# lalithsuresh/rapid

Hardware: NVIDIA H100
Metric: alert_cells_per_sec_to_converged_cut (higher is better)
Workload: dtype u16

## Files before the change

rapid_b200/csrc/cd_bucketed.cu:

```cuda
#include <cooperative_groups.h>

#include <algorithm>
#include <climits>
#include <cstdlib>

#include "cd_internal.cuh"

namespace cg = cooperative_groups;

namespace rapid {

#ifndef RAPID_UNI_MINBLOCKS
#define RAPID_UNI_MINBLOCKS 5
#endif
#ifndef RAPID_SPLIT_LOOP
#define RAPID_SPLIT_LOOP 0
#endif
#ifndef RAPID_PF
#define RAPID_PF 2
#endif
#ifndef RAPID_INVAL_SPLIT
#define RAPID_INVAL_SPLIT 1
#endif
#ifndef RAPID_PF_L1
// ... 472 lines not shown
                    }
                    s_ne[t] = (uint8_t)ne;
                }
                if (fresh && !edges) {
                    un = (visit_acc<PERM, SEQ>(f, 0u, d, &sw[0], &spw[0], RM, L, H) && block_active) ? 1 : 0;
                    if (PERM) { f.minTH = T32_NONE; f.minTLun = T32_NONE; }
                } else {
                    if (!PERM) sw[t] = a.walk[base + t];
                    if (SEQ) spw[t] = a.pwalk[base + t];
                    if (fresh) s_src[t] = nullptr;
                    if (MEMO && !fresh && !edges && block_active) {
                        const uint32_t sst = rows.get(s_src[t], (int64_t)sample_at);
                        uint32_t at_last = sst;
                        const bool mun = visit_acc<PERM, SEQ>(m, sst & RM, d, &sw[PERM ? 0 : t], &spw[SEQ ? t : 0], RM, L, H, nullptr, 0u, seq_last, &at_last);
                        s_mst[t] = sst;
                        s_mrep[t] = group8_rep<HB>((SEQ ? (at_last | (sst & ~RM)) : sst) | s_nw[t]);
                        s_mun[t] = mun ? 1 : 0;
                        memo = true;
                    }
                }
                if (MEMO) { if (!memo) s_mst[t] = 0xFFFFFFFFu; else s_macc[t] = stage_pack<SEQ>(m); }
                s_unres[t] = (un && a.wl.has_so[d.slot]) ? 1 : 0;
                if (!fresh || edges) s_unres[t] = a.wl.has_so[d.slot] ? 0 : -1;
                heavy = !fresh || edges;
            }
            {
                const unsigned hm = __ballot_sync(0xffffffffu, heavy);
                if (t == 0) s_heavy = __popc(hm);
            }
            const StageAcc fr = stage_reduce<SEQ>(stage_pack<SEQ>(f));
            if (t == 0) chunk_add<SEQ>(s_facc, fr);
// ... 70 lines not shown
                        uint32_t so_st = 0;
                        if (s_erow[i][e]) same = group8_same<HB>(group8_load<HB>(rows, s_erow[i][e], r0), am, &so_st);
                        const int ob = s_eob[i][e], k = s_ek[i][e];
                        const uint32_t bLo = observer_L_batch(so_st & RM, ob >= 0 ? &a.desc[ob] : nullptr, ob >= 0 ? &a.pwalk[ob] : nullptr, L);
                        u[k] = (bLo == T32_NONE || bDown == T32_NONE) ? T32_NONE : max(bLo, bDown);
                        umask |= 1u << k;
                    }
                }
                if (mhit) {
                    hit |= 1u << i;
                    unres = s_mun[i] != 0;
                    group8_merge<HB>(w, s_mrep[i], am);
                } else if (same) {
                    uint32_t at_last = st;
                    unres = visit_acc<PERM, SEQ>(com, st & RM, d, &sw[PERM ? 0 : i], &spw[SEQ ? i : 0], RM, L, H, u, umask, seq_last, &at_last);
                    group8_merge<HB>(w, group8_rep<HB>((SEQ ? (at_last | (st & ~RM)) : st) | s_nw[i]), am);
                } else {
                    if (!had_exc) {
                        had_exc = true;
                        const Acc zero;
#pragma unroll
                        for (int j = 0; j < 8; ++j) part_store<SEQ>(a.part, pbase + j, zero);
                    }
                    const uint32_t nwb = s_nw[i];
#pragma unroll (SEQ ? 1 : 8)
                    for (int j = 0; j < 8; ++j) {
                        if (!((act >> j) & 1u)) continue;
                        const uint32_t sj = group8_word<HB>(w, j);
                        Acc ex;
                        uint32_t at_last = sj;
                        if (SEQ && ne) umask = edge_times(a, d.slot, r0 + j, false, receiver_down_batch(a, ((seen >> j) & 1u) ? RF_SEEN_DOWN : 0u, false), u);
// ... 170 lines not shown
                    if (v.seen_down) fl |= PF_SEEN;
                    if (v.c0 >= L && v.c0 < H) tp++;
                    if (v.crossL) nL++;
                    if (v.crossH) {
                        nH++;
                        if (!haveTH || v.tH < minTH) { minTH = v.tH; haveTH = true; }
                        h1 += d.mix1; h2 += d.mix2;
                    }
                    if (v.c1 >= L && v.c1 < H) {
                        unres = true;
                        if (v.crossL) { nUn++; if (!haveTL || v.tL < minTLun) { minTLun = v.tL; haveTL = true; } }
                        else fl |= PF_NEGINF;
                    }
                    st |= v.have;
                }
                if (a.rows.hb == 4) row_store1_warp<4>(a.rows, s_dst[i], r, st);
                else row_store1_warp<8>(a.rows, s_dst[i], r, st);
            }
            if (__any_sync(0xffffffffu, unres) && (t & 31) == 0 && s_unres[i] == 0) s_unres[i] = 1;
        }
        __syncthreads();
        if (t < n && s_unres[t] > 0) note_unresolved(a, tile, sd[t].slot);
    }
    if (t == 0) {
        if ((blockIdx.x * GEN_THREADS) % TILE_R == 0) a.part.flag[(size_t)chunk * a.part.n_tiles + tile] = 1;
        if (blockIdx.x == 0) a.part.chunk[chunk] = chunk_zero();
    }
    if (r < (int64_t)a.Rpad) {
        const size_t p = (size_t)chunk * a.Rpad + (size_t)r;
        a.part.cnt[p] = make_uint4(nL, nH, tp | (fl << PF_SHIFT), nUn);
        a.part.minTH[p] = minTH;
        a.part.minTLun[p] = minTLun;
        a.part.h1[p] = h1;
        a.part.h2[p] = h2;
    }
}

struct ResolveArgs {
    ApplyArgs ap;
    BatchCounts* bc;
    BatchCounts* snap;
    int n_chunks;
    int uniform;
    int counts_only;
    int seq;
    uint8_t* seq_dev;
    uint8_t* cur_w;
    int32_t* n_pre;
    uint32_t* rflags;
    uint64_t* pend_h1;
    uint64_t* pend_h2;
    int32_t* pend_cnt;
    uint64_t* out_h1;
    uint64_t* out_h2;
// ... 291 lines not shown
    for (int64_t r = (int64_t)blockIdx.x * blockDim.x + threadIdx.x; r < a.ap.R; r += (int64_t)gridDim.x * blockDim.x) {
        const uint32_t fl = a.mx_fl[r];
        if (!((fl & MX_DONE) && (fl & MX_HAS_E))) continue;
        const uint64_t o1 = a.mx_p1[r] + a.mx_e1[r], o2 = a.mx_p2[r] + a.mx_e2[r];
        const int32_t oc = a.mx_pc[r] + a.mx_ec[r];
        a.out_h1[r] = o1; a.out_h2[r] = o2; a.out_len[r] = oc;
        a.pend_h1[r] -= o1; a.pend_h2[r] -= o2; a.pend_cnt[r] -= oc;
        a.mx_e1[r] = 0; a.mx_e2[r] = 0; a.mx_ec[r] = 0;
        a.rflags[r] = (a.rflags[r] | RF_ANNOUNCED | RF_ANN_NOW | RF_MIXED_EMIT) & ~RF_RULE_GE_H;
    }
}

__device__ __noinline__ bool emitted_in_batch(const ResolveArgs& e, int32_t s, int64_t r, uint32_t w_new, uint64_t rs) {
    const ApplyArgs& a = e.ap;
    const uint32_t RM = (1u << a.K) - 1u;
    if (e.touch[s] != e.serial) return __popc(w_new & RM) >= a.H && !(w_new & CD_BIT_CALL);
    const int b = e.batch_index[s];
    const SubjDesc d = a.desc[b];
    const uint32_t old = seq_state(a, d, b, r, (s >= a.bc->S_before ? 0u : a.rows.get(a.rows.alt_lo(s), r)) & RM, true, true);
    if (__popc(old & RM) >= a.H) return true;
    SubjWalk wl;
    if (e.uniform) wl = a.walk[b];
    const IVisit v = interval_visit(a, e.uniform, old & RM, d, &wl, r, rs);
    return v.crossH && v.tH <= e.estar[r];
}

constexpr int INV_STAGE = 128;
struct InvSmem {
    uint8_t* row[INV_STAGE];
    uint64_t mix1[INV_STAGE], mix2[INV_STAGE];
    uint8_t ne[INV_STAGE];
// ... 96 lines not shown
                            miss[j] = (k3[j] && c >= a.L && c < a.H) ? (~w[j] & RM) : 0u;
                            anymiss |= miss[j];
                        }
                        if (!anymiss) continue;
                        uint32_t implicit[4] = {0u, 0u, 0u, 0u};
                        for (int ei = eb; ei < ee; ++ei) {
                            const int k = sm.e_k[ei];
                            if (!((anymiss >> k) & 1u)) continue;
                            const uint2 o2 = ei == eb ? e0v[q] : ei == eb + 1 ? e1v[q] : a.rows.load4(sm.e_row[ei], rb);
                            uint32_t wo[4];
#pragma unroll
                            for (int j = 0; j < 4; ++j) wo[j] = a.rows.word4(o2, j);
#pragma unroll
                            for (int j = 0; j < 4; ++j) {
                                if (!((miss[j] >> k) & 1u)) continue;
                                if ((wo[j] & CD_BIT_EMIT) || __popc(wo[j] & RM) < a.L) continue;
                                if (MX) {
                                    const int64_t r = rb + j;
                                    if (emitted_in_batch(e, sm.e_so[ei], r, wo[j], splitmix64(a.dl.perm_seed + (uint64_t)(a.rbegin + r)))) continue;
                                }
                                implicit[j] |= 1u << k;
                            }
                        }
                        bool any = false;
#pragma unroll
                        for (int j = 0; j < 4; ++j) {
                            if (!implicit[j]) continue;
                            any = true;
                            uint32_t nw = w[j] | implicit[j];
                            const bool raised = __popc(nw & RM) >= a.H;
                            if (raised && mixed) nw |= CD_BIT_CALL;
                            w[j] = nw;
                            if (raised) { ++res[j]; kh1[j] += sm.mix1[i]; kh2[j] += sm.mix2[i]; }
                        }
                        if (any) a.rows.store4(sm.row[i], rb, w);
                    }
                }
            }
        }
#if RAPID_INVAL_SPLIT
        if (P > 1) {
#pragma unroll
            for (int j = 0; j < 4; ++j)
                if (res[j] > 0) { atomicAdd(&e.inv_res[rb + j], res[j]); atomicAdd(&e.inv_h1[rb + j], (unsigned long long)kh1[j]); atomicAdd(&e.inv_h2[rb + j], (unsigned long long)kh2[j]); }
            __threadfence();
            __syncthreads();
            if (t == 0) s_fin = atomicAdd(&e.inv_ticket[tile], 1) == P - 1 ? 1 : 0;
            __syncthreads();
            if (!s_fin) continue;
// ... 31 lines not shown
            if ((flags[j] & RF_MIXED_EMIT) && (flags[j] & RF_ANN_NOW) && !(flags[j] & RF_RULE_GE_H)) ++my_inval;
            ann |= ((flags[j] & RF_ANNOUNCED) ? 1u : 0u) << (8 * j);
        }
        if (touched) {
            *reinterpret_cast<uint4*>(e.rflags + rb) = make_uint4(flags[0], flags[1], flags[2], flags[3]);
            *reinterpret_cast<uint32_t*>(e.out_ann + rb) = ann;
        }
    }
    if (MX) {
        const int32_t b = block_sum_i32(my_inval, s_red);
        if (t == 0 && b) atomicAdd(&e.bc->n_inval, b);
    }
}

__device__ __noinline__ void phase_mixed_mark(const ResolveArgs& e, int32_t S) {
    const ApplyArgs& a = e.ap;
    const int spb = 64;
    const int rblocks = (int)(a.Rpad / GEN_THREADS), sblocks = (S + spb - 1) / spb;
    const int64_t items = (int64_t)rblocks * sblocks;
    for (int64_t wi = blockIdx.x; wi < items; wi += gridDim.x) {
        const int64_t r = (wi % rblocks) * GEN_THREADS + threadIdx.x;
        if (r >= a.R) continue;
        const uint32_t f = e.rflags[r];
        if (!(f & RF_MIXED_EMIT) || !(f & RF_ANN_NOW) || (f & RF_RULE_GE_H)) continue;
        const uint64_t rs = splitmix64(a.dl.perm_seed + (uint64_t)(a.rbegin + r));
        const int32_t s0 = (int32_t)(wi / rblocks) * spb, s1 = min(S, s0 + spb);
        for (int32_t s = s0; s < s1; ++s) {
            uint8_t* row = a.rows.cur_lo(s);
            const uint32_t w = a.rows.get(row, r);
            if (!(w & CD_BIT_EMIT) && emitted_in_batch(e, s, r, w, rs)) a.rows.hi_or(row, r, CD_BIT_EMIT);
        }
    }
}

__device__ void phase_inval_unmark(const ResolveArgs& e) {
    const ApplyArgs& a = e.ap;
    const int n_list = min(*(volatile int32_t*)a.wl.count, a.wl.cap);
    const int64_t items = (int64_t)n_list * a.wl.n_tiles;
    for (int64_t p = blockIdx.x; p < items; p += gridDim.x) {
        const int32_t sl = a.wl.slots[p / a.wl.n_tiles];
        const int tile = (int)(p % a.wl.n_tiles);
        if (!a.wl.in_tile[(size_t)sl * a.wl.n_tiles + tile]) continue;
        uint8_t* row = a.rows.cur_lo(sl);
        for (int q = 0; q < TILE_R / GEN_THREADS; ++q) {
            const int64_t r = (int64_t)tile * TILE_R + q * GEN_THREADS + threadIdx.x;
            if (r >= a.R) continue;
            if (a.rows.get(row, r) & CD_BIT_CALL) a.rows.hi_clear(row, r, CD_BIT_CALL);
        }
    }
}

__device__ void resolve_tail(const ResolveArgs& a, int32_t serial) {
    __shared__ int s_last;
    __syncthreads();
    if (threadIdx.x == 0) {
        __threadfence();
        s_last = atomicAdd(&a.bc->ticket, 1) == (int)gridDim.x - 1;
    }
    __syncthreads();
    if (!s_last || threadIdx.x != 0) return;
    __threadfence();
    volatile BatchCounts* b = a.bc;
    BatchCounts c;
// ... 368 lines not shown
    }
}

int32_t bucketed_apply(CD* cd, int64_t A, const DeliveryDev& dl, bool seq) {
    Bucketed* b = state(cd);
    cudaStream_t s = cd->stream;
    const bool uniform = !(dl.flags & (RAPID_DELIVERY_BITMAP | RAPID_DELIVERY_PERMUTED));
    const bool counts_only = (dl.flags & RAPID_DELIVERY_PERMUTED) && !(dl.flags & RAPID_DELIVERY_BITMAP);
    const bool swar = uniform || counts_only;
    b->n_tiles = (int)(cd->Rpad / TILE_R);

    if (b->slots_uniform == 0) {
        int dev = 0, sms = TARGET_SMS, per_u = 8, per_g = 4, per_r = 2;
        cudaGetDevice(&dev);
        cudaDeviceGetAttribute(&sms, cudaDevAttrMultiProcessorCount, dev);
        cudaOccupancyMaxActiveBlocksPerMultiprocessor(&per_u, k_apply_uniform<false, false, 4>, UNI_THREADS, 0);
        cudaOccupancyMaxActiveBlocksPerMultiprocessor(&per_g, k_apply_generic, GEN_THREADS, 0);
        cudaOccupancyMaxActiveBlocksPerMultiprocessor(&per_r, k_mixed_flip, GEN_THREADS, 0);
        int per_m = 2;
        cudaOccupancyMaxActiveBlocksPerMultiprocessor(&per_m, k_marks, GEN_THREADS, 0);
        per_r = std::min(per_r, per_m);
        b->slots_uniform = sms * std::max(per_u, 1);
        b->slots_generic = sms * std::max(per_g, 1);
        b->resolve_grid = sms * std::max(per_r, 1);
    }
    int Sb = (int)std::max<int64_t>(1, std::min<int64_t>(A, cd->est_A > 0 ? (A * (int64_t)std::max(cd->est_Sb, 1) + cd->est_A - 1) / cd->est_A
                                                                           : (2 * A + cd->K - 1) / cd->K));
    Sb = (int)std::min<int64_t>(Sb, (int64_t)std::max<size_t>(cd->S_cap, 1));
    int n_chunks = 1;
    {
        const int rblocks = swar ? b->n_tiles : (int)(cd->Rpad / GEN_THREADS);
// ... 37 lines not shown
    RAPID_CHECK(b->p_chunk.reserve((size_t)n_chunks));
    Partials part{b->p_cnt.p, b->p_cntp.p, b->p_minTH.p, b->p_minTLun.p, b->p_h1.p, b->p_h2.p, b->p_h1p.p, b->p_h2p.p, b->p_seq.p, b->p_flag.p, b->p_chunk.p, b->n_tiles};

    ApplyArgs ap;
    ap.rows = RowRef{cd->masks.p, cd->cur.p, cd->Rpad, cd->row_stride, cd->nbuf, cd->hb}; ap.Rpad = cd->Rpad;
    ap.K = cd->K; ap.H = cd->H; ap.L = cd->L; ap.R = cd->R; ap.rbegin = cd->rbegin;
    ap.rflags = cd->rflags.p; ap.dl = dl; ap.bc = cd->counts.p;
    ap.desc = b->desc.p; ap.walk = b->walk.p; ap.pwalk = b->pwalk.p; ap.slot_subject = cd->slot_subject.p;
    ap.touch = cd->touch.p; ap.batch_index = b->batch_index.p; ap.serial = cd->batch_serial; ap.seq = seq ? 1 : 0;
    ap.sidx = b->sidx.p; ap.s_ring = b->s_ring.p; ap.s_status = b->s_status.p;
    ap.part = part; ap.n_tiles = b->n_tiles; ap.wl = worklist(b);

    RAPID_CUDA(cudaEventRecord(cd->evk0, s));
    if (swar) {
        dim3 grid((unsigned)b->n_tiles, (unsigned)n_chunks);
        if (cd->hb == 4) launch_uniform<4>(grid, s, ap, counts_only, seq);
        else launch_uniform<8>(grid, s, ap, counts_only, seq);
        cd->last_path = counts_only ? 4 : 2;
    } else {
        dim3 grid((unsigned)(cd->Rpad / GEN_THREADS), (unsigned)n_chunks);
        k_apply_generic<<<grid, GEN_THREADS, 0, s>>>(ap);
        cd->last_path = 3;
    }
    RAPID_KERNEL_CHECK();
    RAPID_CUDA(cudaEventRecord(cd->evk1, s));

    ResolveArgs ra;
    ra.ap = ap; ra.bc = cd->counts.p; ra.snap = cd->counts_snap.p; ra.n_chunks = n_chunks;
    ra.uniform = uniform ? 1 : 0; ra.counts_only = counts_only ? 1 : 0; ra.cur_w = cd->cur.p;
    ra.seq = seq ? 1 : 0; ra.seq_dev = nullptr;
    ra.n_pre = cd->n_pre.p; ra.rflags = cd->rflags.p; ra.pend_h1 = cd->pend_h1.p; ra.pend_h2 = cd->pend_h2.p;
    ra.pend_cnt = cd->pend_cnt.p; ra.out_h1 = cd->out_h1.p; ra.out_h2 = cd->out_h2.p; ra.out_len = cd->out_len.p; ra.out_ann = cd->out_ann.p;
    ra.mx_fl = b->mx_fl.p; ra.mx_a = b->mx_a.p; ra.mx_cand = b->mx_cand.p; ra.mx_emax = b->mx_emax.p;
    ra.mx_p1 = b->mx_p1.p; ra.mx_p2 = b->mx_p2.p; ra.mx_pc = b->mx_pc.p; ra.estar = b->estar.p;
    ra.mx_e1 = b->mx_e1.p; ra.mx_e2 = b->mx_e2.p; ra.mx_ec = b->mx_ec.p; ra.mx_changed = b->mx_changed.p; ra.mx_dev = b->mx_dev.p;
    ra.slot_of = cd->slot_of.p; ra.obs = cd->view->obs.p; ra.touch = cd->touch.p; ra.batch_index = b->batch_index.p;
    ra.serial = cd->batch_serial;
#if RAPID_INVAL_SPLIT
    const int inv_split = b->n_tiles >= 64 ? 1 : std::min(32, (2 * TARGET_SMS + std::max(b->n_tiles, 1) - 1) / std::max(b->n_tiles, 1));
    if (inv_split > 1 && !b->inv_res.p) {
        RAPID_CHECK(b->inv_res.reserve(cd->Rpad)); RAPID_CHECK(b->inv_h1.reserve(cd->Rpad)); RAPID_CHECK(b->inv_h2.reserve(cd->Rpad));
        RAPID_CHECK(b->inv_ticket.reserve((size_t)std::max(b->n_tiles, 1)));
        RAPID_CUDA(cudaMemsetAsync(b->inv_res.p, 0, cd->Rpad * sizeof(int32_t), s));
// ... 35 lines not shown
```

rapid_b200/csrc/cd_core.cu:

```cuda
#include <algorithm>
#include <climits>
#include <cstdio>
#include <cstdlib>

#include "cd_internal.cuh"
#include "radix.cuh"

namespace rapid {

__global__ void k_fill_i32(int32_t* p, int64_t n, int32_t v) {
    const int64_t i = (int64_t)blockIdx.x * blockDim.x + threadIdx.x;
    if (i < n) p[i] = v;
}

struct SweepArgs {
    int K, H, L, raw, do_cells, do_inval;
    int64_t R;
    RowRef rows;
    int32_t S;
    const int32_t* slot_subject;
    const int32_t* slot_of;
    const int32_t* obs;
    int64_t A;
    const int32_t* cell_slot;
// ... 127 lines not shown
    if (w & CD_BIT_CALL) {
        *p = (uint16_t)(w & ~CD_BIT_CALL);
        const int32_t at = atomicAdd(count, 1);
        if (at < cap) out[at] = slot_subject[s];
    }
}
__global__ void k_clear_call(RowRef rows, int32_t S, int64_t R) {
    const int64_t r = (int64_t)blockIdx.x * blockDim.x + threadIdx.x;
    const int32_t s = blockIdx.y;
    if (r >= R || s >= S) return;
    uint16_t* p = rows.row(s) + r;
    const uint32_t w = *p;
    if (w & CD_BIT_CALL) *p = (uint16_t)(w & ~CD_BIT_CALL);
}

__global__ void k_gather_proposal(RowRef rows, int32_t S, int64_t r, int H, uint32_t RM, int rule_ge_h,
                                  const int32_t* __restrict__ slot_subject, const int64_t* __restrict__ key0,
                                  int32_t* __restrict__ out_ids, int64_t* __restrict__ out_keys, int32_t cap,
                                  int32_t* __restrict__ count) {
    const int32_t s = blockIdx.x * blockDim.x + threadIdx.x;
    if (s >= S) return;
    const uint32_t w = rows.get(s, r);
    const bool in = rule_ge_h ? (__popc(w & RM) >= H) : ((w & CD_BIT_EMIT) != 0);
    if (in) {
        const int32_t at = atomicAdd(count, 1);
        if (at < cap) { const int32_t id = slot_subject[s]; out_ids[at] = id; out_keys[at] = key0[id]; }
    }
}

__global__ void k_dump_masks(RowRef rows, int32_t S, int64_t r, uint32_t RM, const int32_t* __restrict__ slot_subject,
                             int32_t* __restrict__ out_ids, uint16_t* __restrict__ out_masks) {
    const int32_t s = blockIdx.x * blockDim.x + threadIdx.x;
    if (s >= S) return;
    out_ids[s] = slot_subject[s];
    out_masks[s] = (uint16_t)(rows.get(s, r) & RM);
}

__global__ void k_reset_slots(int32_t S, const BatchCounts* __restrict__ bc, const int32_t* __restrict__ slot_subject,
// ... 3 lines not shown
    if (s < S) { slot_of[slot_subject[s]] = -1; cur[s] = 0; }
}

__global__ void k_clear_receivers(int64_t R, int32_t* __restrict__ n_pre, int32_t* __restrict__ n_prop, uint32_t* __restrict__ rflags,
                                  uint64_t* __restrict__ pend_h1, uint64_t* __restrict__ pend_h2, int32_t* __restrict__ pend_cnt,
                                  uint64_t* __restrict__ out_h1, uint64_t* __restrict__ out_h2, int32_t* __restrict__ out_len,
                                  uint8_t* __restrict__ out_ann) {
    const int64_t r = (int64_t)blockIdx.x * blockDim.x + threadIdx.x;
    if (r >= R) return;
    n_pre[r] = 0; n_prop[r] = 0; rflags[r] = 0u;
    pend_h1[r] = 0; pend_h2[r] = 0; pend_cnt[r] = 0;
    out_h1[r] = 0; out_h2[r] = 0; out_len[r] = 0; out_ann[r] = 0;
}

static RowRef rowref(const CD* cd) { return RowRef{cd->masks.p, cd->cur.p, cd->Rpad, cd->row_stride, cd->nbuf, cd->hb}; }

static int32_t ensure_id_capacity(CD* cd) {
    const int64_t ntot = cd->view->n + cd->view->nj;
    if (ntot <= cd->ntot_cap) return RAPID_OK;
    int64_t ncap = std::max<int64_t>(cd->ntot_cap, 64);
    while (ncap < ntot) ncap *= 2;
    const int64_t old = cd->ntot_cap;
    RAPID_CHECK(cd->slot_of.reserve((size_t)ncap, true, cd->stream));
    RAPID_CHECK(cd->first_idx.reserve((size_t)ncap, true, cd->stream));
    RAPID_CHECK(cd->slot_subject.reserve((size_t)ncap, true, cd->stream));
    RAPID_CHECK(cd->touch.reserve((size_t)ncap, true, cd->stream));
    ncap = (int64_t)std::min(std::min(cd->slot_of.cap, cd->touch.cap), std::min(cd->first_idx.cap, cd->slot_subject.cap));
    const int TB = 256;
    k_fill_i32<<<(unsigned)ceil_div<int64_t>(ncap - old, TB), TB, 0, cd->stream>>>(cd->slot_of.p + old, ncap - old, -1);
    k_fill_i32<<<(unsigned)ceil_div<int64_t>(ncap - old, TB), TB, 0, cd->stream>>>(cd->first_idx.p + old, ncap - old, INT_MAX);
// ... 5 lines not shown

static int32_t ensure_slot_capacity(CD* cd, size_t need) {
    if (need <= cd->S_cap) return RAPID_OK;
    size_t ncap = need;
    if (cd->S_cap) { ncap = cd->S_cap; while (ncap < need) ncap *= 2; }
    const size_t row = cd->row_stride * (size_t)cd->nbuf;
    const size_t old_bytes = cd->S_cap * row;
    DevBuf<uint8_t> nm;
    RAPID_CHECK(nm.reserve(ncap * row));
    if (old_bytes) RAPID_CUDA(cudaMemcpyAsync(nm.p, cd->masks.p, old_bytes, cudaMemcpyDeviceToDevice, cd->stream));
    RAPID_CUDA(cudaMemsetAsync(nm.p + old_bytes, 0, ncap * row - old_bytes, cd->stream));
    DevBuf<uint8_t> nc;
    RAPID_CHECK(nc.reserve(ncap));
    RAPID_CUDA(cudaMemsetAsync(nc.p, 0, ncap, cd->stream));
    if (cd->S_cap) RAPID_CUDA(cudaMemcpyAsync(nc.p, cd->cur.p, cd->S_cap, cudaMemcpyDeviceToDevice, cd->stream));
    RAPID_CUDA(cudaStreamSynchronize(cd->stream));
    std::swap(cd->masks.p, nm.p); std::swap(cd->masks.cap, nm.cap);
    std::swap(cd->cur.p, nc.p); std::swap(cd->cur.cap, nc.cap);
    cd->S_cap = ncap;
    return RAPID_OK;
}

static int32_t preprocess(CD* cd, int64_t cfg, int64_t A, const int32_t* dst_dev, const uint8_t* ring_dev,
                          const uint8_t* status_dev, const int64_t* cfg_dev, BatchCounts* out) {
    cudaStream_t s = cd->stream;
    RAPID_CHECK(ensure_id_capacity(cd));
    RAPID_CHECK(cd->cell_slot.reserve(std::max<int64_t>(A, 1)));
    BatchCounts init;
    memset(&init, 0, sizeof(init));
    init.n_slots = cd->S;
    cd->S_before = cd->S;
    init.bad_ring = -1;
    init.bad_dst = -1;
// ... 832 lines not shown
    if (!cd || !out_len || receiver < 0 || receiver >= cd->R) { set_error("bad arguments"); return RAPID_EINVAL; }
    DeviceGuard g(cd->device);
    RAPID_CHECK(cd_wait(cd, false));
    uint32_t flags = 0;
    RAPID_CUDA(cudaMemcpy(&flags, cd->rflags.p + receiver, sizeof(flags), cudaMemcpyDeviceToHost));
    *out_len = 0;
    if (!(flags & RF_ANNOUNCED) || cd->S == 0) return RAPID_OK;
    DevBuf<int32_t> d_ids, d_cnt;
    DevBuf<int64_t> d_keys;
    const int32_t S = cd->S;
    RAPID_CHECK(d_ids.reserve((size_t)S));
    RAPID_CHECK(d_keys.reserve((size_t)S));
    RAPID_CHECK(d_cnt.reserve(1));
    RAPID_CUDA(cudaMemsetAsync(d_cnt.p, 0, sizeof(int32_t), cd->stream));
    k_gather_proposal<<<(unsigned)ceil_div<int32_t>(S, 256), 256, 0, cd->stream>>>(
        rowref(cd), S, receiver, cd->H, (1u << cd->K) - 1u, (flags & RF_RULE_GE_H) ? 1 : 0, cd->slot_subject.p, cd->view->key.p ,
        d_ids.p, d_keys.p, S, d_cnt.p);
    RAPID_KERNEL_CHECK();
    int32_t n = 0;
    RAPID_CUDA(cudaMemcpyAsync(&n, d_cnt.p, sizeof(int32_t), cudaMemcpyDeviceToHost, cd->stream));
    RAPID_CUDA(cudaStreamSynchronize(cd->stream));
    std::vector<int32_t> ids;
    std::vector<int64_t> keys;
    RAPID_CHECK(gather_sorted(cd, n, ids, &keys, d_ids, &d_keys));
    std::vector<int32_t> order((size_t)n);
    for (int32_t i = 0; i < n; ++i) order[(size_t)i] = i;
    std::sort(order.begin(), order.end(), [&](int32_t a, int32_t b) {
        return keys[(size_t)a] != keys[(size_t)b] ? keys[(size_t)a] < keys[(size_t)b] : ids[(size_t)a] < ids[(size_t)b];
    });
    *out_len = n;
    for (int32_t i = 0; i < n && i < cap; ++i) out_ids[i] = ids[(size_t)order[(size_t)i]];
// ... 87 lines not shown
```

rapid_b200/csrc/cd_internal.cuh:

```cuda
#pragma once

#include <string>
#include <type_traits>
#include <vector>

#include "common.cuh"

namespace rapid {

#define CD_BIT_CALL 0x4000u
#define CD_BIT_EMIT 0x8000u

#define RF_SEEN_DOWN   1u
#define RF_ANNOUNCED   2u
#define RF_RULE_GE_H   4u
#define RF_ANN_NOW     8u

struct BatchCounts {
    int32_t n_slots;
    int32_t n_valid;
    int32_t n_batch_subj;
    int32_t any_down;
    int32_t bad_ring;
    int32_t bad_dst;
// ... 23 lines not shown
    cudaEvent_t ev0 = nullptr, ev1 = nullptr, evk0 = nullptr, evk1 = nullptr;
    int K = 0, H = 0, L = 0;
    uint32_t mode = 0;
    bool raw = false, bucketed = false;
    int64_t R = 0, rbegin = 0;
    size_t Rpad = 0;
    int nbuf = 1;
    int32_t S = 0;
    int32_t S_before = 0;
    size_t S_cap = 0;
    int64_t ntot_cap = 0;

    int hb = 0;
    size_t row_stride = 0;
    DevBuf<uint8_t> masks;
    DevBuf<uint8_t> cur;
    DevBuf<int32_t> slot_of;
    DevBuf<int32_t> first_idx;
    DevBuf<int32_t> slot_subject;
    DevBuf<int32_t> touch;
    int32_t batch_serial = 0;
    int prep_grid_max = 0;

    DevBuf<int32_t> n_pre;
    DevBuf<int32_t> n_prop;
    DevBuf<uint32_t> rflags;
    DevBuf<uint64_t> pend_h1, pend_h2;
    DevBuf<int32_t> pend_cnt;
    DevBuf<uint64_t> out_h1, out_h2;
    DevBuf<int64_t> batch_off;
// ... 28 lines not shown
    int32_t deferred_rc = 0;
    std::string deferred_msg;
    int32_t est_Sb = 0;
    int64_t est_A = 0;
    BatchCounts last;
    int32_t retries = 0;
    DevBuf<unsigned long long> prep_stamps;
    void* bucketed_state = nullptr;

    int32_t last_path = 0, last_launches = 0;
    int32_t last_chunks = 0, last_prep_grid = 0;
    float last_ms = 0.f, last_main_ms = 0.f;
    int64_t last_A = 0;
};

__host__ __device__ inline int row_hi_bits(int K) { return K <= 10 ? 4 : 8; }

template <int HB>
__device__ __forceinline__ uint32_t hi_pack(uint32_t w) {
    return HB == 4 ? (((w >> 8) & 3u) | ((w >> 12) & 0xCu)) : ((w >> 8) & 0xFFu);
}
template <int HB>
__device__ __forceinline__ uint32_t hi_unpack(uint32_t h) {
    return HB == 4 ? (((h & 3u) << 8) | ((h & 0xCu) << 12)) : (h << 8);
}

struct RowRef {
    uint8_t* base;
    const uint8_t* cur;
    size_t Rpad;
    size_t stride;
    int nbuf;
    int hb;

    __device__ __forceinline__ uint8_t* lo(int32_t slot, int buf) const { return base + ((size_t)slot * nbuf + buf) * stride; }
    __device__ __forceinline__ uint8_t* cur_lo(int32_t slot) const { return lo(slot, nbuf == 2 ? cur[slot] : 0); }
    __device__ __forceinline__ uint8_t* alt_lo(int32_t slot) const { return lo(slot, cur[slot] ^ 1); }
    __device__ __forceinline__ uint16_t* row(int32_t slot) const {
        return reinterpret_cast<uint16_t*>(cur_lo(slot));
    }

    __device__ __forceinline__ uint32_t get(const uint8_t* l, int64_t r) const {
        if (hb == 0) return reinterpret_cast<const uint16_t*>(l)[r];
        if (hb == 4) return l[r] | hi_unpack<4>((l[Rpad + (r >> 1)] >> ((r & 1) * 4)) & 0xFu);
        return l[r] | hi_unpack<8>(l[Rpad + r]);
    }
    __device__ __forceinline__ uint32_t get(int32_t slot, int64_t r) const { return get(cur_lo(slot), r); }

    __device__ __forceinline__ uint2 load4(const uint8_t* l, int64_t r) const {
        return make_uint2(*reinterpret_cast<const uint32_t*>(l + r),
                          hb == 4 ? (uint32_t)*reinterpret_cast<const uint16_t*>(l + Rpad + (r >> 1))
                                  : *reinterpret_cast<const uint32_t*>(l + Rpad + r));
    }
    __device__ __forceinline__ uint32_t word4(uint2 g, int j) const {
        return ((g.x >> (8 * j)) & 0xFFu) | (hb == 4 ? hi_unpack<4>((g.y >> (4 * j)) & 0xFu) : hi_unpack<8>((g.y >> (8 * j)) & 0xFFu));
    }
    __device__ __forceinline__ void store4(uint8_t* l, int64_t r, const uint32_t w[4]) const {
        uint32_t lw = 0, hw = 0;
#pragma unroll
        for (int j = 0; j < 4; ++j) {
            lw |= (w[j] & 0xFFu) << (8 * j);
            hw |= hb == 4 ? hi_pack<4>(w[j]) << (4 * j) : hi_pack<8>(w[j]) << (8 * j);
        }
        *reinterpret_cast<uint32_t*>(l + r) = lw;
        if (hb == 4) *reinterpret_cast<uint16_t*>(l + Rpad + (r >> 1)) = (uint16_t)hw;
        else *reinterpret_cast<uint32_t*>(l + Rpad + r) = hw;
    }

    __device__ __forceinline__ uint32_t* hi_word(uint8_t* l, int64_t r, uint32_t bit, uint32_t* shift) const {
        const int64_t p = r * hb + (hb - (bit == CD_BIT_EMIT ? 1 : 2));
        *shift = (uint32_t)(p & 31);
        return reinterpret_cast<uint32_t*>(l + Rpad) + (p >> 5);
    }
    __device__ __forceinline__ void hi_or(uint8_t* l, int64_t r, uint32_t bit) const {
        uint32_t sh;
        uint32_t* p = hi_word(l, r, bit, &sh);
        atomicOr(p, 1u << sh);
    }
    __device__ __forceinline__ void hi_clear(uint8_t* l, int64_t r, uint32_t bit) const {
        uint32_t sh;
        uint32_t* p = hi_word(l, r, bit, &sh);
        atomicAnd(p, ~(1u << sh));
    }
};

template <int HB>
struct Group8 {
    using Hi = typename std::conditional<HB == 4, uint32_t, uint64_t>::type;
    uint64_t lo;
    Hi hi;
};
template <int HB>
__device__ __forceinline__ const uint8_t* group8_hi(const RowRef& rows, const uint8_t* l, int64_t r) {
    return l + rows.Rpad + (r * HB >> 3);
}
template <int HB>
__device__ __forceinline__ Group8<HB> group8_load(const RowRef& rows, const uint8_t* l, int64_t r) {
    Group8<HB> g;
    g.lo = *reinterpret_cast<const uint64_t*>(l + r);
    g.hi = *reinterpret_cast<const typename Group8<HB>::Hi*>(group8_hi<HB>(rows, l, r));
    return g;
}
template <int HB>
__device__ __forceinline__ void group8_store(const RowRef& rows, uint8_t* l, int64_t r, const Group8<HB>& g) {
    *reinterpret_cast<uint64_t*>(l + r) = g.lo;
    *reinterpret_cast<typename Group8<HB>::Hi*>(const_cast<uint8_t*>(group8_hi<HB>(rows, l, r))) = g.hi;
}
template <int HB>
__device__ __forceinline__ uint32_t group8_word(const Group8<HB>& g, int j) {
    return (uint32_t)((g.lo >> (8 * j)) & 0xFFu) | hi_unpack<HB>((uint32_t)(g.hi >> (HB * j)) & ((1u << HB) - 1u));
}
template <int HB>
__device__ __forceinline__ void group8_or_word(Group8<HB>& g, int j, uint32_t w) {
    g.lo |= (uint64_t)(w & 0xFFu) << (8 * j);
    g.hi |= (typename Group8<HB>::Hi)hi_pack<HB>(w) << (HB * j);
}
template <int HB>
__device__ __forceinline__ uint2 group8_rep(uint32_t w) {
    return make_uint2((w & 0xFFu) * 0x01010101u, hi_pack<HB>(w) * (HB == 4 ? 0x11111111u : 0x01010101u));
}
template <int HB>
__device__ __forceinline__ Group8<HB> group8_mask(uint32_t act) {
    Group8<HB> m;
    m.lo = 0; m.hi = 0;
#pragma unroll
    for (int j = 0; j < 8; ++j)
        if ((act >> j) & 1u) { m.lo |= 0xFFull << (8 * j); m.hi |= (typename Group8<HB>::Hi)((1u << HB) - 1u) << (HB * j); }
    return m;
}
template <int HB>
__device__ __forceinline__ Group8<HB> group8_fill(uint2 rep, const Group8<HB>& m) {
    Group8<HB> g;
    g.lo = (((uint64_t)rep.x << 32) | rep.x) & m.lo;
    g.hi = (HB == 4 ? (typename Group8<HB>::Hi)rep.y : (typename Group8<HB>::Hi)(((uint64_t)rep.y << 32) | rep.y)) & m.hi;
    return g;
}
template <int HB>
__device__ __forceinline__ void group8_merge(Group8<HB>& g, uint2 rep, const Group8<HB>& m) {
    const Group8<HB> f = group8_fill<HB>(rep, m);
    g.lo = (g.lo & ~m.lo) | f.lo;
    g.hi = (g.hi & ~m.hi) | f.hi;
}
template <int B, typename T>
__device__ __forceinline__ bool lanes_same(T x, T m, uint32_t* v) {
    T a = x | ~m, o = x & m;
#pragma unroll
    for (int s = 4 * B; s >= B; s >>= 1) { a &= a >> s; o |= o >> s; }
    const uint32_t lm = (1u << B) - 1u;
    *v = (uint32_t)o & lm;
    return ((uint32_t)a & lm) == *v;
}
template <int HB>
__device__ __forceinline__ bool group8_same(const Group8<HB>& g, const Group8<HB>& m, uint32_t* st) {
    uint32_t vl, vh;
    const bool sl = lanes_same<8>(g.lo, m.lo, &vl);
    const bool sh = lanes_same<HB>(g.hi, m.hi, &vh);
    *st = vl | hi_unpack<HB>(vh);
    return sl && sh;
}

template <int HB>
__device__ __forceinline__ void row_store1_warp(const RowRef& rows, uint8_t* l, int64_t r, uint32_t w) {
    l[r] = (uint8_t)w;
    if (HB == 8) {
        l[rows.Rpad + r] = (uint8_t)hi_pack<8>(w);
    } else {
        uint32_t h = hi_pack<4>(w) << (4 * (r & 7));
        h |= __shfl_xor_sync(0xffffffffu, h, 1);
        h |= __shfl_xor_sync(0xffffffffu, h, 2);
        h |= __shfl_xor_sync(0xffffffffu, h, 4);
        if ((r & 7) == 0) *reinterpret_cast<uint32_t*>(l + rows.Rpad + (r >> 1)) = h;
    }
}

struct DeliveryDev {
    uint32_t flags = 0;
    const uint8_t* blocked = nullptr;
    const uint32_t* bitmap = nullptr;
    int64_t words = 0;
    uint64_t perm_seed = 0;
    int64_t cell_base = 0;
};

struct SubjDesc {
    int32_t slot;
    uint16_t bmask;
    uint8_t nr;
    uint8_t any_down;
// ... 65 lines not shown
```

Measured before the change: 18.04 million.

## Move emit/call flags to separate bit planes and shrink row high bits to two

The per-cell EMIT and CALL flag bits move out of the packed row words into separate per-slot bitmask planes (emit_marks, trans_marks), so the row high-bits field for K<=10 narrows from 4 to 2 bits per cell. The apply kernels then stream fewer bytes per row. Mixed-mark writes become warp-ballot word stores and invalidation clears plane words directly instead of doing per-cell atomics. The cost is extra plane memory, extra atomics and loads on the resolve path, and more complicated growth and copy logic for the new buffers.

Result: faster. 20.55 million (median of 6 runs) (+13.9%).

```diff
diff --git a/profiles/roofline_rows.py b/profiles/roofline_rows.py
--- /dev/null
+++ b/profiles/roofline_rows.py
@@ -0,0 +1,59 @@
+import json
+import re
+import sys
+
+TILE = 1024
+EXTRA_PER_RECEIVER = 5
+
+
+def row_bytes(K, path):
+    if path == "sweep":
+        return 2.0
+    return 1.0 + (2 if K <= 10 else 8) / 8.0
+
+
+def padded(R, path):
+    return R if path == "sweep" else -(-R // TILE) * TILE
+
+
+def true_bytes(line):
+    cfg = line["config"]
+    K, R, path = cfg["K"], cfg["receivers_per_gpu"], cfg.get("kernel_path", "bucketed-uniform")
+    rb, Rp = row_bytes(K, path), padded(R, path)
+    out = {}
+    rl = line["roofline"]
+    if rl.get("per_batch"):
+        fresh = sum(b["fresh_subjects"] for b in rl["per_batch"])
+        carried = sum(b["carried_subjects"] for b in rl["per_batch"])
+    else:
+        fresh, carried = cfg["subjects"], 0
+    launches = rl.get("launches_per_step", 1)
+    alg = (rb * fresh + 2 * rb * carried) * Rp + EXTRA_PER_RECEIVER * R * launches
+    out["roofline"] = (alg / launches, rl["kernel_ms"], rl["peak"])
+    rc = line.get("roofline_carried")
+    if rc:
+        m = re.search(r"(\d+) carried subjects.*?(\d+) fresh", rc["kernel"])
+        sc, sf = int(m.group(1)), int(m.group(2))
+        alg2 = (2 * rb * sc + rb * sf) * Rp + EXTRA_PER_RECEIVER * R
+        out["roofline_carried"] = (alg2, rc["kernel_ms"], rc["peak"])
+    return out
+
+
+def main(paths):
+    streams = [open(p) for p in paths] if paths else [sys.stdin]
+    for f in streams:
+        for text in f:
+            text = text.strip()
+            if not text.startswith("{"):
+                continue
+            line = json.loads(text)
+            if "roofline" not in line:
+                continue
+            print(line["config"]["workload"])
+            for name, (alg, ms, peak) in true_bytes(line).items():
+                tbs = alg / (ms * 1e-3) / 1e12
+                print("  %-16s %7.3f GB per launch  %7.3f ms  %5.2f TB/s  %.2f of %.2f TB/s" % (name, alg / 1e9, ms, tbs, tbs * 1e3 / peak, peak / 1e3))
+
+
+if __name__ == "__main__":
+    main(sys.argv[1:])
diff --git a/rapid_b200/csrc/cd_bucketed.cu b/rapid_b200/csrc/cd_bucketed.cu
--- a/rapid_b200/csrc/cd_bucketed.cu
+++ b/rapid_b200/csrc/cd_bucketed.cu
@@ -510,7 +510,7 @@
                         uint32_t at_last = sst;
                         const bool mun = visit_acc<PERM, SEQ>(m, sst & RM, d, &sw[PERM ? 0 : t], &spw[SEQ ? t : 0], RM, L, H, nullptr, 0u, seq_last, &at_last);
                         s_mst[t] = sst;
-                        s_mrep[t] = group8_rep<HB>((SEQ ? (at_last | (sst & ~RM)) : sst) | s_nw[t]);
+                        s_mrep[t] = group8_rep<HB>((SEQ ? at_last : sst) | s_nw[t]);
                         s_mun[t] = mun ? 1 : 0;
                         memo = true;
                     }
@@ -611,7 +611,7 @@
                 } else if (same) {
                     uint32_t at_last = st;
                     unres = visit_acc<PERM, SEQ>(com, st & RM, d, &sw[PERM ? 0 : i], &spw[SEQ ? i : 0], RM, L, H, u, umask, seq_last, &at_last);
-                    group8_merge<HB>(w, group8_rep<HB>((SEQ ? (at_last | (st & ~RM)) : st) | s_nw[i]), am);
+                    group8_merge<HB>(w, group8_rep<HB>((SEQ ? at_last : st) | s_nw[i]), am);
                 } else {
                     if (!had_exc) {
                         had_exc = true;
@@ -812,7 +812,7 @@
                     }
                     st |= v.have;
                 }
-                if (a.rows.hb == 4) row_store1_warp<4>(a.rows, s_dst[i], r, st);
+                if (a.rows.hb == 2) row_store1_warp<2>(a.rows, s_dst[i], r, st);
                 else row_store1_warp<8>(a.rows, s_dst[i], r, st);
             }
             if (__any_sync(0xffffffffu, unres) && (t & 31) == 0 && s_unres[i] == 0) s_unres[i] = 1;
@@ -836,6 +836,8 @@
 
 struct ResolveArgs {
     ApplyArgs ap;
+    MarkPlane emit;
+    MarkPlane trans;
     BatchCounts* bc;
     BatchCounts* snap;
     int n_chunks;
@@ -1157,7 +1159,7 @@
 __device__ __noinline__ bool emitted_in_batch(const ResolveArgs& e, int32_t s, int64_t r, uint32_t w_new, uint64_t rs) {
     const ApplyArgs& a = e.ap;
     const uint32_t RM = (1u << a.K) - 1u;
-    if (e.touch[s] != e.serial) return __popc(w_new & RM) >= a.H && !(w_new & CD_BIT_CALL);
+    if (e.touch[s] != e.serial) return __popc(w_new & RM) >= a.H && !e.trans.test(s, r);
     const int b = e.batch_index[s];
     const SubjDesc d = a.desc[b];
     const uint32_t old = seq_state(a, d, b, r, (s >= a.bc->S_before ? 0u : a.rows.get(a.rows.alt_lo(s), r)) & RM, true, true);
@@ -1284,7 +1286,7 @@
 #pragma unroll
                             for (int j = 0; j < 4; ++j) {
                                 if (!((miss[j] >> k) & 1u)) continue;
-                                if ((wo[j] & CD_BIT_EMIT) || __popc(wo[j] & RM) < a.L) continue;
+                                if (__popc(wo[j] & RM) < a.L) continue;
                                 if (MX) {
                                     const int64_t r = rb + j;
                                     if (emitted_in_batch(e, sm.e_so[ei], r, wo[j], splitmix64(a.dl.perm_seed + (uint64_t)(a.rbegin + r)))) continue;
@@ -1293,16 +1295,17 @@
                             }
                         }
                         bool any = false;
+                        uint32_t trans = 0;
 #pragma unroll
                         for (int j = 0; j < 4; ++j) {
                             if (!implicit[j]) continue;
                             any = true;
-                            uint32_t nw = w[j] | implicit[j];
-                            const bool raised = __popc(nw & RM) >= a.H;
-                            if (raised && mixed) nw |= CD_BIT_CALL;
-                            w[j] = nw;
+                            w[j] |= implicit[j];
+                            const bool raised = __popc(w[j] & RM) >= a.H;
+                            if (raised && mixed) trans |= 1u << j;
                             if (raised) { ++res[j]; kh1[j] += sm.mix1[i]; kh2[j] += sm.mix2[i]; }
                         }
+                        if (trans) atomicOr(e.trans.word(a.wl.slots[base + i], rb), trans << (rb & 31));
                         if (any) a.rows.store4(sm.row[i], rb, w);
                     }
                 }
@@ -1364,21 +1367,26 @@
 }
 
 __device__ __noinline__ void phase_mixed_mark(const ResolveArgs& e, int32_t S) {
+    static_assert(GEN_THREADS % 32 == 0, "a warp owns one word of the plane");
     const ApplyArgs& a = e.ap;
     const int spb = 64;
     const int rblocks = (int)(a.Rpad / GEN_THREADS), sblocks = (S + spb - 1) / spb;
     const int64_t items = (int64_t)rblocks * sblocks;
     for (int64_t wi = blockIdx.x; wi < items; wi += gridDim.x) {
         const int64_t r = (wi % rblocks) * GEN_THREADS + threadIdx.x;
-        if (r >= a.R) continue;
-        const uint32_t f = e.rflags[r];
-        if (!(f & RF_MIXED_EMIT) || !(f & RF_ANN_NOW) || (f & RF_RULE_GE_H)) continue;
+        const uint32_t f = r < a.R ? e.rflags[r] : 0u;
+        const bool marked = (f & RF_MIXED_EMIT) && (f & RF_ANN_NOW) && !(f & RF_RULE_GE_H);
+        const uint32_t mm = __ballot_sync(0xffffffffu, marked);
+        if (mm == 0) continue;
         const uint64_t rs = splitmix64(a.dl.perm_seed + (uint64_t)(a.rbegin + r));
         const int32_t s0 = (int32_t)(wi / rblocks) * spb, s1 = min(S, s0 + spb);
         for (int32_t s = s0; s < s1; ++s) {
-            uint8_t* row = a.rows.cur_lo(s);
-            const uint32_t w = a.rows.get(row, r);
-            if (!(w & CD_BIT_EMIT) && emitted_in_batch(e, s, r, w, rs)) a.rows.hi_or(row, r, CD_BIT_EMIT);
+            const bool em = marked && emitted_in_batch(e, s, r, a.rows.get(s, r), rs);
+            const uint32_t b = __ballot_sync(0xffffffffu, em);
+            if ((threadIdx.x & 31) == 0) {
+                uint32_t* p = e.emit.word(s, r);
+                *p = (*p & ~mm) | b;
+            }
         }
     }
 }
@@ -1386,17 +1394,14 @@
 __device__ void phase_inval_unmark(const ResolveArgs& e) {
     const ApplyArgs& a = e.ap;
     const int n_list = min(*(volatile int32_t*)a.wl.count, a.wl.cap);
-    const int64_t items = (int64_t)n_list * a.wl.n_tiles;
-    for (int64_t p = blockIdx.x; p < items; p += gridDim.x) {
+    constexpr int TW = TILE_R / 32;
+    const int64_t items = (int64_t)n_list * a.wl.n_tiles * TW;
+    for (int64_t q = (int64_t)blockIdx.x * blockDim.x + threadIdx.x; q < items; q += (int64_t)gridDim.x * blockDim.x) {
+        const int64_t p = q / TW;
         const int32_t sl = a.wl.slots[p / a.wl.n_tiles];
         const int tile = (int)(p % a.wl.n_tiles);
         if (!a.wl.in_tile[(size_t)sl * a.wl.n_tiles + tile]) continue;
-        uint8_t* row = a.rows.cur_lo(sl);
-        for (int q = 0; q < TILE_R / GEN_THREADS; ++q) {
-            const int64_t r = (int64_t)tile * TILE_R + q * GEN_THREADS + threadIdx.x;
-            if (r >= a.R) continue;
-            if (a.rows.get(row, r) & CD_BIT_CALL) a.rows.hi_clear(row, r, CD_BIT_CALL);
-        }
+        e.trans.p[(size_t)sl * e.trans.words + (size_t)tile * TW + (size_t)(q % TW)] = 0u;
     }
 }
 
@@ -1795,7 +1800,7 @@
         int dev = 0, sms = TARGET_SMS, per_u = 8, per_g = 4, per_r = 2;
         cudaGetDevice(&dev);
         cudaDeviceGetAttribute(&sms, cudaDevAttrMultiProcessorCount, dev);
-        cudaOccupancyMaxActiveBlocksPerMultiprocessor(&per_u, k_apply_uniform<false, false, 4>, UNI_THREADS, 0);
+        cudaOccupancyMaxActiveBlocksPerMultiprocessor(&per_u, k_apply_uniform<false, false, 2>, UNI_THREADS, 0);
         cudaOccupancyMaxActiveBlocksPerMultiprocessor(&per_g, k_apply_generic, GEN_THREADS, 0);
         cudaOccupancyMaxActiveBlocksPerMultiprocessor(&per_r, k_mixed_flip, GEN_THREADS, 0);
         int per_m = 2;
@@ -1863,7 +1868,7 @@
     RAPID_CUDA(cudaEventRecord(cd->evk0, s));
     if (swar) {
         dim3 grid((unsigned)b->n_tiles, (unsigned)n_chunks);
-        if (cd->hb == 4) launch_uniform<4>(grid, s, ap, counts_only, seq);
+        if (cd->hb == 2) launch_uniform<2>(grid, s, ap, counts_only, seq);
         else launch_uniform<8>(grid, s, ap, counts_only, seq);
         cd->last_path = counts_only ? 4 : 2;
     } else {
@@ -1875,7 +1880,8 @@
     RAPID_CUDA(cudaEventRecord(cd->evk1, s));
 
     ResolveArgs ra;
-    ra.ap = ap; ra.bc = cd->counts.p; ra.snap = cd->counts_snap.p; ra.n_chunks = n_chunks;
+    ra.ap = ap; ra.bc = cd->counts.p;
+    ra.emit = MarkPlane{cd->emit_marks.p, cd->Rpad / 32}; ra.trans = MarkPlane{cd->trans_marks.p, cd->Rpad / 32}; ra.snap = cd->counts_snap.p; ra.n_chunks = n_chunks;
     ra.uniform = uniform ? 1 : 0; ra.counts_only = counts_only ? 1 : 0; ra.cur_w = cd->cur.p;
     ra.seq = seq ? 1 : 0; ra.seq_dev = nullptr;
     ra.n_pre = cd->n_pre.p; ra.rflags = cd->rflags.p; ra.pend_h1 = cd->pend_h1.p; ra.pend_h2 = cd->pend_h2.p;
diff --git a/rapid_b200/csrc/cd_core.cu b/rapid_b200/csrc/cd_core.cu
--- a/rapid_b200/csrc/cd_core.cu
+++ b/rapid_b200/csrc/cd_core.cu
@@ -165,14 +165,15 @@
     if (w & CD_BIT_CALL) *p = (uint16_t)(w & ~CD_BIT_CALL);
 }
 
-__global__ void k_gather_proposal(RowRef rows, int32_t S, int64_t r, int H, uint32_t RM, int rule_ge_h,
+__global__ void k_gather_proposal(RowRef rows, MarkPlane emit, int32_t S, int64_t r, int H, uint32_t RM, int rule_ge_h,
                                   const int32_t* __restrict__ slot_subject, const int64_t* __restrict__ key0,
                                   int32_t* __restrict__ out_ids, int64_t* __restrict__ out_keys, int32_t cap,
                                   int32_t* __restrict__ count) {
     const int32_t s = blockIdx.x * blockDim.x + threadIdx.x;
     if (s >= S) return;
     const uint32_t w = rows.get(s, r);
-    const bool in = rule_ge_h ? (__popc(w & RM) >= H) : ((w & CD_BIT_EMIT) != 0);
+    const bool ge_h = __popc(w & RM) >= H;
+    const bool in = rule_ge_h ? ge_h : emit.p ? (ge_h && emit.test(s, r)) : ((w & CD_BIT_EMIT) != 0);
     if (in) {
         const int32_t at = atomicAdd(count, 1);
         if (at < cap) { const int32_t id = slot_subject[s]; out_ids[at] = id; out_keys[at] = key0[id]; }
@@ -206,6 +207,7 @@
 }
 
 static RowRef rowref(const CD* cd) { return RowRef{cd->masks.p, cd->cur.p, cd->Rpad, cd->row_stride, cd->nbuf, cd->hb}; }
+static MarkPlane emit_plane(const CD* cd) { return MarkPlane{cd->bucketed ? cd->emit_marks.p : nullptr, cd->Rpad / 32}; }
 
 static int32_t ensure_id_capacity(CD* cd) {
     const int64_t ntot = cd->view->n + cd->view->nj;
@@ -241,9 +243,25 @@
     RAPID_CHECK(nc.reserve(ncap));
     RAPID_CUDA(cudaMemsetAsync(nc.p, 0, ncap, cd->stream));
     if (cd->S_cap) RAPID_CUDA(cudaMemcpyAsync(nc.p, cd->cur.p, cd->S_cap, cudaMemcpyDeviceToDevice, cd->stream));
+    const size_t words = cd->Rpad / 32, old_words = cd->S_cap * words;
+    auto grow_plane = [&](const DevBuf<uint32_t>& from, DevBuf<uint32_t>& to) -> int32_t {
+        RAPID_CHECK(to.reserve(ncap * words));
+        if (old_words) RAPID_CUDA(cudaMemcpyAsync(to.p, from.p, old_words * sizeof(uint32_t), cudaMemcpyDeviceToDevice, cd->stream));
+        RAPID_CUDA(cudaMemsetAsync(to.p + old_words, 0, (ncap * words - old_words) * sizeof(uint32_t), cd->stream));
+        return RAPID_OK;
+    };
+    DevBuf<uint32_t> ne, nt;
+    if (cd->bucketed) {
+        RAPID_CHECK(grow_plane(cd->emit_marks, ne));
+        RAPID_CHECK(grow_plane(cd->trans_marks, nt));
+    }
     RAPID_CUDA(cudaStreamSynchronize(cd->stream));
     std::swap(cd->masks.p, nm.p); std::swap(cd->masks.cap, nm.cap);
     std::swap(cd->cur.p, nc.p); std::swap(cd->cur.cap, nc.cap);
+    if (cd->bucketed) {
+        std::swap(cd->emit_marks.p, ne.p); std::swap(cd->emit_marks.cap, ne.cap);
+        std::swap(cd->trans_marks.p, nt.p); std::swap(cd->trans_marks.cap, nt.cap);
+    }
     cd->S_cap = ncap;
     return RAPID_OK;
 }
@@ -1106,7 +1124,7 @@
     RAPID_CHECK(d_cnt.reserve(1));
     RAPID_CUDA(cudaMemsetAsync(d_cnt.p, 0, sizeof(int32_t), cd->stream));
     k_gather_proposal<<<(unsigned)ceil_div<int32_t>(S, 256), 256, 0, cd->stream>>>(
-        rowref(cd), S, receiver, cd->H, (1u << cd->K) - 1u, (flags & RF_RULE_GE_H) ? 1 : 0, cd->slot_subject.p, cd->view->key.p ,
+        rowref(cd), emit_plane(cd), S, receiver, cd->H, (1u << cd->K) - 1u, (flags & RF_RULE_GE_H) ? 1 : 0, cd->slot_subject.p, cd->view->key.p ,
         d_ids.p, d_keys.p, S, d_cnt.p);
     RAPID_KERNEL_CHECK();
     int32_t n = 0;
diff --git a/rapid_b200/csrc/cd_internal.cuh b/rapid_b200/csrc/cd_internal.cuh
--- a/rapid_b200/csrc/cd_internal.cuh
+++ b/rapid_b200/csrc/cd_internal.cuh
@@ -61,6 +61,8 @@
     int hb = 0;
     size_t row_stride = 0;
     DevBuf<uint8_t> masks;
+    DevBuf<uint32_t> emit_marks;
+    DevBuf<uint32_t> trans_marks;
     DevBuf<uint8_t> cur;
     DevBuf<int32_t> slot_of;
     DevBuf<int32_t> first_idx;
@@ -119,15 +121,14 @@
     int64_t last_A = 0;
 };
 
-__host__ __device__ inline int row_hi_bits(int K) { return K <= 10 ? 4 : 8; }
+__host__ __device__ inline int row_hi_bits(int K) { return K <= 10 ? 2 : 8; }
 
 template <int HB>
 __device__ __forceinline__ uint32_t hi_pack(uint32_t w) {
-    return HB == 4 ? (((w >> 8) & 3u) | ((w >> 12) & 0xCu)) : ((w >> 8) & 0xFFu);
-}
-template <int HB>
+    return (w >> 8) & ((1u << HB) - 1u);
+}
 __device__ __forceinline__ uint32_t hi_unpack(uint32_t h) {
-    return HB == 4 ? (((h & 3u) << 8) | ((h & 0xCu) << 12)) : (h << 8);
+    return h << 8;
 }
 
 struct RowRef {
@@ -147,51 +148,34 @@
 
     __device__ __forceinline__ uint32_t get(const uint8_t* l, int64_t r) const {
         if (hb == 0) return reinterpret_cast<const uint16_t*>(l)[r];
-        if (hb == 4) return l[r] | hi_unpack<4>((l[Rpad + (r >> 1)] >> ((r & 1) * 4)) & 0xFu);
-        return l[r] | hi_unpack<8>(l[Rpad + r]);
+        if (hb == 2) return l[r] | hi_unpack((l[Rpad + (r >> 2)] >> ((r & 3) * 2)) & 3u);
+        return l[r] | hi_unpack(l[Rpad + r]);
     }
     __device__ __forceinline__ uint32_t get(int32_t slot, int64_t r) const { return get(cur_lo(slot), r); }
 
     __device__ __forceinline__ uint2 load4(const uint8_t* l, int64_t r) const {
         return make_uint2(*reinterpret_cast<const uint32_t*>(l + r),
-                          hb == 4 ? (uint32_t)*reinterpret_cast<const uint16_t*>(l + Rpad + (r >> 1))
-                                  : *reinterpret_cast<const uint32_t*>(l + Rpad + r));
+                          hb == 2 ? (uint32_t)l[Rpad + (r >> 2)] : *reinterpret_cast<const uint32_t*>(l + Rpad + r));
     }
     __device__ __forceinline__ uint32_t word4(uint2 g, int j) const {
-        return ((g.x >> (8 * j)) & 0xFFu) | (hb == 4 ? hi_unpack<4>((g.y >> (4 * j)) & 0xFu) : hi_unpack<8>((g.y >> (8 * j)) & 0xFFu));
+        return ((g.x >> (8 * j)) & 0xFFu) | hi_unpack(hb == 2 ? (g.y >> (2 * j)) & 3u : (g.y >> (8 * j)) & 0xFFu);
     }
     __device__ __forceinline__ void store4(uint8_t* l, int64_t r, const uint32_t w[4]) const {
         uint32_t lw = 0, hw = 0;
 #pragma unroll
         for (int j = 0; j < 4; ++j) {
             lw |= (w[j] & 0xFFu) << (8 * j);
-            hw |= hb == 4 ? hi_pack<4>(w[j]) << (4 * j) : hi_pack<8>(w[j]) << (8 * j);
+            hw |= hb == 2 ? hi_pack<2>(w[j]) << (2 * j) : hi_pack<8>(w[j]) << (8 * j);
         }
         *reinterpret_cast<uint32_t*>(l + r) = lw;
-        if (hb == 4) *reinterpret_cast<uint16_t*>(l + Rpad + (r >> 1)) = (uint16_t)hw;
+        if (hb == 2) l[Rpad + (r >> 2)] = (uint8_t)hw;
         else *reinterpret_cast<uint32_t*>(l + Rpad + r) = hw;
     }
-
-    __device__ __forceinline__ uint32_t* hi_word(uint8_t* l, int64_t r, uint32_t bit, uint32_t* shift) const {
-        const int64_t p = r * hb + (hb - (bit == CD_BIT_EMIT ? 1 : 2));
-        *shift = (uint32_t)(p & 31);
-        return reinterpret_cast<uint32_t*>(l + Rpad) + (p >> 5);
-    }
-    __device__ __forceinline__ void hi_or(uint8_t* l, int64_t r, uint32_t bit) const {
-        uint32_t sh;
-        uint32_t* p = hi_word(l, r, bit, &sh);
-        atomicOr(p, 1u << sh);
-    }
-    __device__ __forceinline__ void hi_clear(uint8_t* l, int64_t r, uint32_t bit) const {
-        uint32_t sh;
-        uint32_t* p = hi_word(l, r, bit, &sh);
-        atomicAnd(p, ~(1u << sh));
-    }
 };
 
 template <int HB>
 struct Group8 {
-    using Hi = typename std::conditional<HB == 4, uint32_t, uint64_t>::type;
+    using Hi = typename std::conditional<HB == 2, uint16_t, uint64_t>::type;
     uint64_t lo;
     Hi hi;
 };
@@ -213,44 +197,47 @@
 }
 template <int HB>
 __device__ __forceinline__ uint32_t group8_word(const Group8<HB>& g, int j) {
-    return (uint32_t)((g.lo >> (8 * j)) & 0xFFu) | hi_unpack<HB>((uint32_t)(g.hi >> (HB * j)) & ((1u << HB) - 1u));
+    return (uint32_t)((g.lo >> (8 * j)) & 0xFFu) | hi_unpack((uint32_t)(g.hi >> (HB * j)) & ((1u << HB) - 1u));
 }
 template <int HB>
 __device__ __forceinline__ void group8_or_word(Group8<HB>& g, int j, uint32_t w) {
     g.lo |= (uint64_t)(w & 0xFFu) << (8 * j);
-    g.hi |= (typename Group8<HB>::Hi)hi_pack<HB>(w) << (HB * j);
+    using Hi = typename Group8<HB>::Hi;
+    g.hi = (Hi)(g.hi | ((Hi)hi_pack<HB>(w) << (HB * j)));
 }
 template <int HB>
 __device__ __forceinline__ uint2 group8_rep(uint32_t w) {
-    return make_uint2((w & 0xFFu) * 0x01010101u, hi_pack<HB>(w) * (HB == 4 ? 0x11111111u : 0x01010101u));
+    return make_uint2((w & 0xFFu) * 0x01010101u, hi_pack<HB>(w) * (HB == 2 ? 0x55555555u : 0x01010101u));
 }
 template <int HB>
 __device__ __forceinline__ Group8<HB> group8_mask(uint32_t act) {
+    using Hi = typename Group8<HB>::Hi;
     Group8<HB> m;
     m.lo = 0; m.hi = 0;
 #pragma unroll
     for (int j = 0; j < 8; ++j)
-        if ((act >> j) & 1u) { m.lo |= 0xFFull << (8 * j); m.hi |= (typename Group8<HB>::Hi)((1u << HB) - 1u) << (HB * j); }
+        if ((act >> j) & 1u) { m.lo |= 0xFFull << (8 * j); m.hi = (Hi)(m.hi | ((Hi)((1u << HB) - 1u) << (HB * j))); }
     return m;
 }
 template <int HB>
 __device__ __forceinline__ Group8<HB> group8_fill(uint2 rep, const Group8<HB>& m) {
     Group8<HB> g;
     g.lo = (((uint64_t)rep.x << 32) | rep.x) & m.lo;
-    g.hi = (HB == 4 ? (typename Group8<HB>::Hi)rep.y : (typename Group8<HB>::Hi)(((uint64_t)rep.y << 32) | rep.y)) & m.hi;
+    g.hi = (HB == 2 ? (typename Group8<HB>::Hi)rep.y : (typename Group8<HB>::Hi)(((uint64_t)rep.y << 32) | rep.y)) & m.hi;
     return g;
 }
 template <int HB>
 __device__ __forceinline__ void group8_merge(Group8<HB>& g, uint2 rep, const Group8<HB>& m) {
     const Group8<HB> f = group8_fill<HB>(rep, m);
     g.lo = (g.lo & ~m.lo) | f.lo;
-    g.hi = (g.hi & ~m.hi) | f.hi;
+    g.hi = (typename Group8<HB>::Hi)((g.hi & ~m.hi) | f.hi);
 }
 template <int B, typename T>
 __device__ __forceinline__ bool lanes_same(T x, T m, uint32_t* v) {
-    T a = x | ~m, o = x & m;
+    static_assert(B == (int)sizeof(T), "8 lanes of B bits fill the word");
+    T a = (T)(x | ~m), o = (T)(x & m);
 #pragma unroll
-    for (int s = 4 * B; s >= B; s >>= 1) { a &= a >> s; o |= o >> s; }
+    for (int s = 4 * B; s >= B; s >>= 1) { a &= (T)(a >> s); o |= (T)(o >> s); }
     const uint32_t lm = (1u << B) - 1u;
     *v = (uint32_t)o & lm;
     return ((uint32_t)a & lm) == *v;
@@ -260,7 +247,7 @@
     uint32_t vl, vh;
     const bool sl = lanes_same<8>(g.lo, m.lo, &vl);
     const bool sh = lanes_same<HB>(g.hi, m.hi, &vh);
-    *st = vl | hi_unpack<HB>(vh);
+    *st = vl | hi_unpack(vh);
     return sl && sh;
 }
 
@@ -270,13 +257,21 @@
     if (HB == 8) {
         l[rows.Rpad + r] = (uint8_t)hi_pack<8>(w);
     } else {
-        uint32_t h = hi_pack<4>(w) << (4 * (r & 7));
+        uint32_t h = hi_pack<2>(w) << (2 * (r & 15));
         h |= __shfl_xor_sync(0xffffffffu, h, 1);
         h |= __shfl_xor_sync(0xffffffffu, h, 2);
         h |= __shfl_xor_sync(0xffffffffu, h, 4);
-        if ((r & 7) == 0) *reinterpret_cast<uint32_t*>(l + rows.Rpad + (r >> 1)) = h;
-    }
-}
+        h |= __shfl_xor_sync(0xffffffffu, h, 8);
+        if ((r & 15) == 0) *reinterpret_cast<uint32_t*>(l + rows.Rpad + (r >> 2)) = h;
+    }
+}
+
+struct MarkPlane {
+    uint32_t* p;
+    size_t words;
+    __device__ __forceinline__ uint32_t* word(int32_t slot, int64_t r) const { return p + (size_t)slot * words + (size_t)(r >> 5); }
+    __device__ __forceinline__ bool test(int32_t slot, int64_t r) const { return (*word(slot, r) >> (r & 31)) & 1u; }
+};
 
 struct DeliveryDev {
     uint32_t flags = 0;
```
